# icdm-adteam/MoCoPCI

Measured on AMD Instinct MI355X. Metric: interpolated frames/sec, higher is better.
Workload: dtype f32 (fused MLP layers: fp32 products as 6 bf16-MFMA partials of an exact 3-way split, fp32 accumulate; index paths exact f32)

## Files before the change

mocopci_amd/csrc/cross.hip:

```cpp
#include "common.h"
#include "mfma_split.h"

#ifdef MCP_CROSS_DIAG
__device__ unsigned long long g_cross_diag[8];
#define CROSS_STAMP(slot)                                                                            \
    do {                                                                                             \
        unsigned long long t_;                                                                       \
        __builtin_amdgcn_sched_barrier(0);                                                           \
        asm volatile("s_memtime %0\n\ts_waitcnt lgkmcnt(0)" : "=s"(t_)::"memory");                   \
        __builtin_amdgcn_sched_barrier(0);                                                           \
        if (blockIdx.x == 0 && blockIdx.y == 0 && threadIdx.x == 0) g_cross_diag[slot] += t_ - t_prev; \
        t_prev = t_;                                                                                 \
    } while (0)
#else
#define CROSS_STAMP(slot)
#endif

namespace {

typedef float f32x16 __attribute__((ext_vector_type(16)));
constexpr int KNB = 32;
constexpr float SLOPE = 0.1f;
constexpr int MAX_MAPPED_BATCH = 1024;

__device__ __forceinline__ int chan_of(int r, int h) { return (r & 3) + 8 * (r >> 2) + 4 * h; }
__device__ __forceinline__ float leaky(float v) { return mcp_max_raw(v, v * SLOPE); }

template <int CTRL>
__device__ __forceinline__ float dppf(float v) {
    return __uint_as_float(mcp_dpp<CTRL>(__float_as_uint(v)));
}
#define MCP_MAX_DPP(dst, src0, src1, CTRL)                                                                              \
    asm("s_nop 1\n\tv_max_f32_dpp %0, %1, %2 " CTRL : "+v"(dst) : "v"(src0), "v"(src1))

__device__ __forceinline__ float scatter_max(const f32x16 &acc, int lane) {
    float v8[8], v4[4], v2[2];
#pragma unroll
    for (int r = 0; r < 8; ++r) {
        const auto sw = __builtin_amdgcn_permlane16_swap(__float_as_uint(acc[r]), __float_as_uint(acc[r + 8]), false, false);
        const float a = __uint_as_float(sw[0]), b = __uint_as_float(sw[1]);
        asm("v_max_f32 %0, %1, %2" : "=v"(v8[r]) : "v"(a), "v"(b));
    }
#pragma unroll
    for (int r = 0; r < 4; ++r) {
        float d = v8[r + 4];
        MCP_MAX_DPP(d, v8[r], v8[r], "row_ror:8 row_mask:0xf bank_mask:0x3");
        MCP_MAX_DPP(d, v8[r + 4], d, "row_ror:8 row_mask:0xf bank_mask:0xc");
        v4[r] = d;
    }
#pragma unroll
    for (int r = 0; r < 2; ++r) {
        float d = v4[r + 2];
        MCP_MAX_DPP(d, v4[r], v4[r], "row_half_mirror row_mask:0xf bank_mask:0x5");
        MCP_MAX_DPP(d, v4[r + 2], d, "row_half_mirror row_mask:0xf bank_mask:0xa");
        v2[r] = d;
    }
    const bool b1 = (lane & 2) != 0;
    float keep = b1 ? v2[1] : v2[0];
    const float send = b1 ? v2[0] : v2[1];
    MCP_MAX_DPP(keep, send, keep, "quad_perm:[2,3,0,1] row_mask:0xf bank_mask:0xf");
    MCP_MAX_DPP(keep, keep, keep, "quad_perm:[1,0,3,2] row_mask:0xf bank_mask:0xf");
    return keep;
}
__device__ __forceinline__ int scatter_reg(int lane) { return ((lane >> 4) & 1) * 8 + ((lane >> 3) & 1) * 4 + ((lane >> 2) & 1) * 2 + ((lane >> 1) & 1); }

template <int D>
struct CrossLds {
    static constexpr int T = D / 32;
    static constexpr bool BF = true;
    static constexpr int W_FLOATS = BF ? T * (2 * T) * 3 * 64 * 4 : T * (T * 16 / 4) * 64 * 4;
    static constexpr int POS_FLOATS = T * 2 * 64;
    static constexpr int B_FLOATS = T * 2 * 16;
    static constexpr int OFF_W = 0, OFF_POS = W_FLOATS, OFF_B = OFF_POS + POS_FLOATS;
    static constexpr int FLOATS = OFF_B + B_FLOATS;
};

template <int D>
__global__ __launch_bounds__(256) void cross_pack_kernel(const float *__restrict__ wpos, const float *__restrict__ bpos,
                                                         const float *__restrict__ wmlp, const float *__restrict__ bmlp,
                                                         float *__restrict__ packed) {
    using L = CrossLds<D>;
    constexpr int T = L::T, KQ = T * 4;
    for (int e = blockIdx.x * 256 + threadIdx.x; e < L::FLOATS; e += gridDim.x * 256) {
        float v;
        if (e < L::OFF_POS) {
            if (L::BF) continue;
            const int j = e & 3, lane = (e >> 2) & 63, q = (e >> 8) % KQ, t = (e >> 8) / KQ;
            const int s = 4 * q + j, tin = s >> 4, r = s & 15;
            v = wmlp[(32 * t + (lane & 31)) * D + 32 * tin + chan_of(r, lane >> 5)];
        } else if (e < L::OFF_B) {
            const int f = e - L::OFF_POS, lane = f & 63, s = (f >> 6) & 1, t = f >> 7;
            const int row = 32 * t + (lane & 31), c = 2 * s + (lane >> 5);
            v = c < 3 ? wpos[row * 3 + c] : bpos[row];
        } else {
            const int f = e - L::OFF_B, r = f & 15, h = (f >> 4) & 1, t = f >> 5;
            v = bmlp[32 * t + chan_of(r, h)];
        }
        packed[e] = v;
    }
    if (L::BF) mcp_split_weights(reinterpret_cast<uint4 *>(packed + L::OFF_W), wmlp, D, T, blockIdx.x * 256 + threadIdx.x, gridDim.x * 256);
}

template <int D>
struct CrossShape {
    static constexpr int NW = D == 128 ? 8 : 4;
    static constexpr int WG_PER_CU = D == 64 ? 3 : 1;
    static constexpr int GRID = D == 64 ? 768 : 256;
};

template <int D, int SPLIT>
__global__ __launch_bounds__(64 * CrossShape<D>::NW, CrossShape<D>::WG_PER_CU) void cross_kernel(long long total, int n1, int n2, const float *__restrict__ xyz1,
                                                           const float *__restrict__ xyz2, const float *__restrict__ points1,
                                                           const float *__restrict__ points2, const int *__restrict__ idx,
                                                           const int *__restrict__ idx2, const int *__restrict__ bmap, int shared,
                                                           const float *__restrict__ packed, float *__restrict__ out) {
    using L = CrossLds<D>;
    constexpr int T = L::T, KQ = T * 4;
    constexpr int WAVES = CrossShape<D>::NW;
    constexpr int TO = T / SPLIT;
    constexpr int WH = L::W_FLOATS / SPLIT, SMALL = L::POS_FLOATS + L::B_FLOATS;
    extern __shared__ __attribute__((aligned(16))) float lds[];
    const int tid = threadIdx.x, split = blockIdx.y;
    static_assert(WH % 4 == 0 && SMALL % 4 == 0, "LDS image is copied as float4");
    for (int e = tid; e < WH / 4; e += 64 * WAVES)
        reinterpret_cast<float4 *>(lds)[e] = reinterpret_cast<const float4 *>(packed + L::OFF_W + (size_t)split * WH)[e];
    for (int e = tid; e < SMALL / 4; e += 64 * WAVES)
        reinterpret_cast<float4 *>(lds + WH)[e] = reinterpret_cast<const float4 *>(packed + L::OFF_POS)[e];
    if (bmap) {
        const int nb = (int)(total / n1);
        for (int e = tid; e < nb; e += 64 * WAVES) reinterpret_cast<int *>(lds + WH + SMALL + WAVES * D)[e] = bmap[e];
    }
    __syncthreads();

    const int lane = tid & 63, wave = tid >> 6, h = lane >> 5, col = lane & 31;
    const float4 *wq = reinterpret_cast<const float4 *>(lds);
    const float *lpos = lds + WH, *lbias = lds + WH + L::POS_FLOATS;
    float *row1_lds = lds + WH + SMALL + wave * D;
    const int *bmap_lds = reinterpret_cast<const int *>(lds + WH + SMALL + WAVES * D);

#ifndef MCP_NO_XCD_MAP
    const bool by_xcd = gridDim.x >= 8 && (gridDim.x & 7) == 0;
#else
    const bool by_xcd = false;
#endif
    const long long chunk = by_xcd ? (total + 7) / 8 : total;
    const long long stride = (long long)(by_xcd ? gridDim.x >> 3 : gridDim.x) * WAVES;
    const long long limit = by_xcd ? min(total, ((long long)(blockIdx.x & 7) + 1) * chunk) : total;
    long long p = by_xcd ? (long long)(blockIdx.x & 7) * chunk + (long long)(blockIdx.x >> 3) * WAVES + wave : (long long)blockIdx.x * WAVES + wave;
    float q2x = 0.f, q2y = 0.f, q2z = 0.f, p1x = 0.f, p1y = 0.f, p1z = 0.f;
    float4 r1 = make_float4(0.f, 0.f, 0.f, 0.f);
    float4 rg[T][4];
    auto mapped = [&](int bb, int flag) -> long long { return (bmap && (shared & flag)) ? (long long)bmap_lds[bb] : (long long)bb; };
    struct Pos { int bb, off; };
    const int stride_b = (int)(stride / n1), stride_o = (int)(stride % n1);
    auto advance = [&](Pos q) {
        q.bb += stride_b;
        q.off += stride_o;
        if (q.off >= n1) { q.off -= n1; ++q.bb; }
        return q;
    };
    auto fetch = [&](long long pp, Pos q, int id) {
        const float *q2 = xyz2 + ((long long)q.bb * n2 + id) * 3;
        q2x = q2[0]; q2y = q2[1]; q2z = q2[2];
        p1x = xyz1[pp * 3 + 0]; p1y = xyz1[pp * 3 + 1]; p1z = xyz1[pp * 3 + 2];
        const float4 *row2 = reinterpret_cast<const float4 *>(points2 + (mapped(q.bb, 2) * n2 + id) * D);
        const float4 *row1 = reinterpret_cast<const float4 *>(points1 + (mapped(q.bb, 1) * n1 + q.off) * D);
        r1 = row1[lane < D / 4 ? lane : 0];
#pragma unroll
        for (int t = 0; t < T; ++t)
#pragma unroll
            for (int g = 0; g < 4; ++g) rg[t][g] = row2[(32 * t + 8 * g + 4 * h) >> 2];
    };
    auto nbr = [&](long long pp, Pos q) {
        if (!idx2) return idx[pp * KNB + col];
        const long long ps = mapped(q.bb, 4) * n1 + q.off;
        return col >= 16 ? idx2[pp * 16 + col - 16] : idx[ps * 16 + col];
    };
    long long pn = p + stride;
    Pos qp{(int)(p / n1), (int)(p % n1)};
    Pos qn = advance(qp), qnn = advance(qn);
    int idn = 0;
    if (p < limit) {
        fetch(p, qp, nbr(p, qp));
        if (pn < limit) idn = nbr(pn, qn);
    }
#ifdef MCP_CROSS_DIAG
    unsigned long long t_prev = 0;
    CROSS_STAMP(7);
#endif
    for (; p < limit; p = pn, pn += stride) {
        CROSS_STAMP(0);
        f32x16 x0[L::BF ? 1 : T];
        McpSplit3 xs[L::BF ? 2 * T : 1];
        const float in0 = h ? q2y - p1y : q2x - p1x, in1 = h ? 1.0f : q2z - p1z;
        if (lane < D / 4) reinterpret_cast<float4 *>(row1_lds)[lane] = r1;
        __builtin_amdgcn_wave_barrier();
#pragma unroll
        for (int t = 0; t < T; ++t) {
            f32x16 acc;
#pragma unroll
            for (int g = 0; g < 4; ++g) {
                const float4 a = reinterpret_cast<const float4 *>(row1_lds)[(32 * t + 8 * g + 4 * h) >> 2];
                acc[4 * g + 0] = a.x; acc[4 * g + 1] = a.y; acc[4 * g + 2] = a.z; acc[4 * g + 3] = a.w;
            }
            acc = __builtin_amdgcn_mfma_f32_32x32x2f32(lpos[(t * 2 + 0) * 64 + lane], in0, acc, 0, 0, 0);
            acc = __builtin_amdgcn_mfma_f32_32x32x2f32(lpos[(t * 2 + 1) * 64 + lane], in1, acc, 0, 0, 0);
#pragma unroll
            for (int g = 0; g < 4; ++g) {
                acc[4 * g + 0] = leaky(acc[4 * g + 0] + rg[t][g].x);
                acc[4 * g + 1] = leaky(acc[4 * g + 1] + rg[t][g].y);
                acc[4 * g + 2] = leaky(acc[4 * g + 2] + rg[t][g].z);
                acc[4 * g + 3] = leaky(acc[4 * g + 3] + rg[t][g].w);
            }
            if (L::BF) {
                xs[L::BF ? 2 * t : 0] = mcp_split_kstep(acc, 0);
                xs[L::BF ? 2 * t + 1 : 0] = mcp_split_kstep(acc, 1);
            } else {
                x0[L::BF ? 0 : t] = acc;
            }
        }
        __builtin_amdgcn_wave_barrier();
        CROSS_STAMP(1);
        if (pn < limit) {
            fetch(pn, qn, idn);
            if (pn + stride < limit) idn = nbr(pn + stride, qnn);
        }
        qn = qnn;
        qnn = advance(qnn);
        CROSS_STAMP(2);
#pragma unroll 1
        for (int tl = 0; tl < TO; ++tl) {
            const int t = TO * split + tl;
            f32x16 acc;
#pragma unroll
            for (int r = 0; r < 16; ++r) acc[r] = lbias[(t * 2 + h) * 16 + r];
            if (L::BF) {
                const uint4 *ws = reinterpret_cast<const uint4 *>(lds) + (size_t)tl * (2 * T) * 3 * 64 + lane;
                acc = mcp_tile_split<(L::BF ? 2 * T : 1)>(ws, xs, acc);
            } else {
#pragma unroll
                for (int q4 = 0; q4 < KQ; ++q4) {
                    const float4 w = wq[(tl * KQ + q4) * 64 + lane];
                    const int tin = L::BF ? 0 : q4 >> 2, r0 = (q4 & 3) * 4;
                    acc = __builtin_amdgcn_mfma_f32_32x32x2f32(w.x, x0[tin][r0 + 0], acc, 0, 0, 0);
                    acc = __builtin_amdgcn_mfma_f32_32x32x2f32(w.y, x0[tin][r0 + 1], acc, 0, 0, 0);
                    acc = __builtin_amdgcn_mfma_f32_32x32x2f32(w.z, x0[tin][r0 + 2], acc, 0, 0, 0);
                    acc = __builtin_amdgcn_mfma_f32_32x32x2f32(w.w, x0[tin][r0 + 3], acc, 0, 0, 0);
                }
            }
            CROSS_STAMP(3);
            const float m = leaky(scatter_max(acc, lane));
            if ((lane & 1) == 0) out[p * D + 32 * t + chan_of(scatter_reg(lane), h)] = m;
            CROSS_STAMP(4);
        }
    }
}

constexpr int X256_T = 8, X256_KS = 16, X256_TILE_U4 = X256_KS * 3 * 64, X256_WAVES = 4;
__global__ __launch_bounds__(64 * X256_WAVES, 1) void cross256_stream_kernel(long long total, int n1, int n2, const float *__restrict__ xyz1,
                                                                          const float *__restrict__ xyz2, const float *__restrict__ points1,
                                                                          const float *__restrict__ points2, const int *__restrict__ idx,
                                                                          const int *__restrict__ idx2, const int *__restrict__ bmap, int shared,
                                                                          const float *__restrict__ packed, float *__restrict__ out) {
    using L = CrossLds<256>;
// ... 167 lines not shown
```

mocopci_amd/csrc/mfma_split.h:

```cpp
#pragma once
#include "common.h"

#ifndef MCP_SPLIT_SCHED_MASK
#define MCP_SPLIT_SCHED_MASK 0x0000
#endif

typedef float mcp_f32x16 __attribute__((ext_vector_type(16)));
typedef __bf16 mcp_bf16x8 __attribute__((ext_vector_type(8)));

__device__ __forceinline__ int mcp_chan_of(int r, int h) { return (r & 3) + 8 * (r >> 2) + 4 * h; }
__device__ __forceinline__ uint32_t mcp_top16(float x) { return __float_as_uint(x) & 0xFFFF0000u; }
__device__ __forceinline__ uint32_t mcp_pack_hi(float even, float odd) {
    return __builtin_amdgcn_perm(__float_as_uint(odd), __float_as_uint(even), 0x07060302u);
}

struct McpSplit3 {
    uint4 p1, p2, p3;
};
__device__ __forceinline__ McpSplit3 mcp_split8(const float *v) {
    float r1[8], r2[8];
#pragma unroll
    for (int i = 0; i < 8; ++i) {
        r1[i] = v[i] - __uint_as_float(mcp_top16(v[i]));
        r2[i] = r1[i] - __uint_as_float(mcp_top16(r1[i]));
    }
    McpSplit3 o;
#ifdef MCP_SPLIT_DIAG_NOSPLIT
    o.p1 = make_uint4(mcp_pack_hi(v[0], v[1]), mcp_pack_hi(v[2], v[3]), mcp_pack_hi(v[4], v[5]), mcp_pack_hi(v[6], v[7]));
    o.p2 = o.p1; o.p3 = o.p1;
    return o;
#endif
    o.p1 = make_uint4(mcp_pack_hi(v[0], v[1]), mcp_pack_hi(v[2], v[3]), mcp_pack_hi(v[4], v[5]), mcp_pack_hi(v[6], v[7]));
    o.p2 = make_uint4(mcp_pack_hi(r1[0], r1[1]), mcp_pack_hi(r1[2], r1[3]), mcp_pack_hi(r1[4], r1[5]), mcp_pack_hi(r1[6], r1[7]));
    o.p3 = make_uint4(mcp_pack_hi(r2[0], r2[1]), mcp_pack_hi(r2[2], r2[3]), mcp_pack_hi(r2[4], r2[5]), mcp_pack_hi(r2[6], r2[7]));
    return o;
}
__device__ __forceinline__ McpSplit3 mcp_split_kstep(const mcp_f32x16 &a, int s) {
    float v[8];
#pragma unroll
    for (int i = 0; i < 8; ++i) v[i] = a[8 * s + i];
    return mcp_split8(v);
}
__device__ __forceinline__ mcp_f32x16 mcp_mfma_bf16(uint4 a, uint4 b, mcp_f32x16 c) {
    return __builtin_amdgcn_mfma_f32_32x32x16_bf16(__builtin_bit_cast(mcp_bf16x8, a), __builtin_bit_cast(mcp_bf16x8, b), c, 0, 0, 0);
}
__device__ __forceinline__ mcp_f32x16 mcp_mfma_split(const uint4 *w, const McpSplit3 &x, mcp_f32x16 acc) {
    const uint4 w1 = w[0], w2 = w[64], w3 = w[128];
    acc = mcp_mfma_bf16(w3, x.p1, acc);
    acc = mcp_mfma_bf16(w1, x.p3, acc);
    acc = mcp_mfma_bf16(w2, x.p2, acc);
    acc = mcp_mfma_bf16(w2, x.p1, acc);
    acc = mcp_mfma_bf16(w1, x.p2, acc);
    acc = mcp_mfma_bf16(w1, x.p1, acc);
    return acc;
}
__device__ __forceinline__ void mcp_relu_split4(const mcp_f32x16 &a, int q, McpSplit3 &o) {
    float v[4], r1[4], r2[4];
#pragma unroll
    for (int i = 0; i < 4; ++i) {
        v[i] = fmaxf(a[4 * q + i], 0.f);
        r1[i] = v[i] - __uint_as_float(mcp_top16(v[i]));
        r2[i] = r1[i] - __uint_as_float(mcp_top16(r1[i]));
    }
    const uint32_t a1 = mcp_pack_hi(v[0], v[1]), b1 = mcp_pack_hi(v[2], v[3]);
    const uint32_t a2 = mcp_pack_hi(r1[0], r1[1]), b2 = mcp_pack_hi(r1[2], r1[3]);
    const uint32_t a3 = mcp_pack_hi(r2[0], r2[1]), b3 = mcp_pack_hi(r2[2], r2[3]);
    if (q & 1) { o.p1.z = a1; o.p1.w = b1; o.p2.z = a2; o.p2.w = b2; o.p3.z = a3; o.p3.w = b3; }
    else       { o.p1.x = a1; o.p1.y = b1; o.p2.x = a2; o.p2.y = b2; o.p3.x = a3; o.p3.y = b3; }
}
template <int NF, class Fill>
__device__ __forceinline__ mcp_f32x16 mcp_kstep_fill(const uint4 &w1, const uint4 &w2, const uint4 &w3, const McpSplit3 &x, mcp_f32x16 acc, Fill fill) {
    fill();
    acc = mcp_mfma_bf16(w3, x.p1, acc);
    acc = mcp_mfma_bf16(w1, x.p3, acc);
    acc = mcp_mfma_bf16(w2, x.p2, acc);
    acc = mcp_mfma_bf16(w2, x.p1, acc);
    acc = mcp_mfma_bf16(w1, x.p2, acc);
    acc = mcp_mfma_bf16(w1, x.p1, acc);
    if constexpr (NF > 0) {
        static_assert(NF <= 30, "at most five fillers per MFMA gap");
#define MCP_GAP(i)                                                                         \
    __builtin_amdgcn_sched_group_barrier(0x008, 1, 0);                                                                                    \
    if constexpr ((NF + 5 - (i)) / 6 > 0) __builtin_amdgcn_sched_group_barrier(0x002, (NF + 5 - (i)) / 6, 0);
        MCP_GAP(0) MCP_GAP(1) MCP_GAP(2) MCP_GAP(3) MCP_GAP(4) MCP_GAP(5)
#undef MCP_GAP
    }
    __builtin_amdgcn_sched_barrier(MCP_SPLIT_SCHED_MASK);
    return acc;
}
template <int KSTEPS>
__device__ __forceinline__ mcp_f32x16 mcp_tile_split(const uint4 *ws, const McpSplit3 *xs, mcp_f32x16 acc) {
    uint4 w1 = ws[0], w2 = ws[64], w3 = ws[128];
#pragma unroll
    for (int s = 0; s < KSTEPS; ++s) {
        uint4 n1 = w1, n2 = w2, n3 = w3;
#ifndef MCP_SPLIT_DIAG_NOLOAD
        if (s + 1 < KSTEPS) {
            const uint4 *nx = ws + (size_t)(s + 1) * 3 * 64;
            n1 = nx[0]; n2 = nx[64]; n3 = nx[128];
        }
#endif
        acc = mcp_mfma_bf16(w3, xs[s].p1, acc);
        acc = mcp_mfma_bf16(w1, xs[s].p3, acc);
        acc = mcp_mfma_bf16(w2, xs[s].p2, acc);
        acc = mcp_mfma_bf16(w2, xs[s].p1, acc);
        acc = mcp_mfma_bf16(w1, xs[s].p2, acc);
        acc = mcp_mfma_bf16(w1, xs[s].p1, acc);
        __builtin_amdgcn_sched_barrier(MCP_SPLIT_SCHED_MASK);
        w1 = n1; w2 = n2; w3 = n3;
    }
    return acc;
}

__device__ __forceinline__ void mcp_split_weights(uint4 *dst, const float *__restrict__ w, int cin, int out_tiles, int first, int stride) {
    const int ksteps = cin / 16;
    for (int e = first; e < out_tiles * ksteps * 64; e += stride) {
        const int lane = e & 63, s = (e >> 6) % ksteps, t = (e >> 6) / ksteps;
        float v[8];
#pragma unroll
        for (int i = 0; i < 8; ++i) v[i] = w[(size_t)(32 * t + (lane & 31)) * cin + 32 * (s >> 1) + mcp_chan_of(8 * (s & 1) + i, lane >> 5)];
        const McpSplit3 sp = mcp_split8(v);
        uint4 *o = dst + (size_t)(t * ksteps + s) * 3 * 64 + lane;
        o[0] = sp.p1;
        o[64] = sp.p2;
        o[128] = sp.p3;
    }
}
```

mocopci_amd/csrc/fusion.hip:

```cpp
#include <stdlib.h>

#include "common.h"
#include "mfma_split.h"

namespace {

typedef float f32x16 __attribute__((ext_vector_type(16)));

constexpr int C1 = 64, C2 = 64, NB = 64;
constexpr int WAVES = 4;


__device__ __forceinline__ int chan_of(int r, int h) { return (r & 3) + 8 * (r >> 2) + 4 * h; }

__device__ __forceinline__ float wave_sum(float v) {
#pragma unroll
    for (int o = 32; o > 0; o >>= 1) v += __shfl_xor(v, o);
    return v;
}
__device__ __forceinline__ float wave_max(float v) {
#pragma unroll
    for (int o = 32; o > 0; o >>= 1) v = fmaxf(v, __shfl_xor(v, o));
    return v;
}

#ifdef MCP_AB
constexpr int OFF_W1 = 0, OFF_W2 = 256, OFF_W3 = OFF_W2 + 4096, OFF_B1 = OFF_W3 + 8192, OFF_B2 = OFF_B1 + 64,
              OFF_B3 = OFF_B2 + 64, LDS_FLOATS = OFF_B3 + 128;
__global__ __launch_bounds__(64 * WAVES, 2) void fusion_kernel(long long total, int n, const float *__restrict__ p1,
                                                            const float *__restrict__ p2, const int *__restrict__ idx, const int *__restrict__ idx2,
                                                            const float *__restrict__ w1, const float *__restrict__ b1,
                                                            const float *__restrict__ w2, const float *__restrict__ b2,
                                                            const float *__restrict__ w3, const float *__restrict__ b3,
                                                            float *__restrict__ out) {
    __shared__ __attribute__((aligned(16))) float lds[LDS_FLOATS];
    const int tid = threadIdx.x;
    for (int e = tid; e < 256; e += 64 * WAVES) {
        const int lane = e & 63, s = (e >> 6) & 1, t = e >> 7;
        lds[OFF_W1 + e] = w1[(32 * t + (lane & 31)) * 4 + 2 * s + (lane >> 5)];
    }
    for (int e = tid; e < 4096; e += 64 * WAVES) {
        const int j = e & 3, lane = (e >> 2) & 63, q = (e >> 8) & 7, t = e >> 11;
        const int s = 4 * q + j, tin = s >> 4, r = s & 15;
        lds[OFF_W2 + e] = w2[(32 * t + (lane & 31)) * C1 + 32 * tin + chan_of(r, lane >> 5)];
    }
    for (int e = tid; e < 8192; e += 64 * WAVES) {
        const int j = e & 3, lane = (e >> 2) & 63, q = (e >> 8) & 7, t = e >> 11;
        const int s = 4 * q + j, tin = s >> 4, r = s & 15;
        lds[OFF_W3 + e] = w3[(32 * t + (lane & 31)) * C2 + 32 * tin + chan_of(r, lane >> 5)];
    }
    for (int e = tid; e < 64; e += 64 * WAVES) {
        const int r = e & 15, h = (e >> 4) & 1, t = e >> 5;
        lds[OFF_B1 + e] = b1[32 * t + chan_of(r, h)];
        lds[OFF_B2 + e] = b2[32 * t + chan_of(r, h)];
    }
    for (int e = tid; e < 128; e += 64 * WAVES) {
        const int r = e & 15, h = (e >> 4) & 1, t = e >> 5;
        lds[OFF_B3 + e] = b3[32 * t + chan_of(r, h)];
    }
    __syncthreads();

    const int lane = tid & 63, wave = tid >> 6, h = lane >> 5, col = lane & 31;
    const float4 *w2q = reinterpret_cast<const float4 *>(lds + OFF_W2);
    const float4 *w3q = reinterpret_cast<const float4 *>(lds + OFF_W3);

    const McpUnits units = mcp_units_by_xcd(total, WAVES);
    for (long long p = units.first + wave; p < units.limit; p += units.stride) {
        const long long bb = mcp_div(p, n, mcp_fits32(total));
        const float cx = p1[p * 3 + 0], cy = p1[p * 3 + 1], cz = p1[p * 3 + 2];
        float score[2], nbx[2], nby[2], nbz[2];
#pragma unroll
        for (int ct = 0; ct < 2; ++ct) {
            const int id = idx2 ? (ct ? idx2 : idx)[p * 32 + col] : idx[p * NB + 32 * ct + col];
            const float *q = p2 + ((long long)bb * n + id) * 3;
            const float x = q[0], y = q[1], z = q[2];
            nbx[ct] = x; nby[ct] = y; nbz[ct] = z;
            const float rx = x - cx, ry = y - cy, rz = z - cz;
            const float dist = sqrtf((rx * rx + ry * ry) + rz * rz);
            const float in0 = h ? ry : rx, in1 = h ? dist : rz;
            f32x16 a1[2];
#pragma unroll
            for (int t = 0; t < 2; ++t) {
                f32x16 acc;
#pragma unroll
                for (int r = 0; r < 16; ++r) acc[r] = lds[OFF_B1 + (t * 2 + h) * 16 + r];
                acc = __builtin_amdgcn_mfma_f32_32x32x2f32(lds[OFF_W1 + (t * 2 + 0) * 64 + lane], in0, acc, 0, 0, 0);
                acc = __builtin_amdgcn_mfma_f32_32x32x2f32(lds[OFF_W1 + (t * 2 + 1) * 64 + lane], in1, acc, 0, 0, 0);
#pragma unroll
                for (int r = 0; r < 16; ++r) acc[r] = fmaxf(acc[r], 0.f);
                a1[t] = acc;
            }
            f32x16 a2[2];
#pragma unroll
            for (int t = 0; t < 2; ++t) {
                f32x16 acc;
#pragma unroll
                for (int r = 0; r < 16; ++r) acc[r] = lds[OFF_B2 + (t * 2 + h) * 16 + r];
#pragma unroll
                for (int q4 = 0; q4 < 8; ++q4) {
                    const float4 w = w2q[(t * 8 + q4) * 64 + lane];
                    const int tin = q4 >> 2, r0 = (q4 & 3) * 4;
                    acc = __builtin_amdgcn_mfma_f32_32x32x2f32(w.x, a1[tin][r0 + 0], acc, 0, 0, 0);
                    acc = __builtin_amdgcn_mfma_f32_32x32x2f32(w.y, a1[tin][r0 + 1], acc, 0, 0, 0);
                    acc = __builtin_amdgcn_mfma_f32_32x32x2f32(w.z, a1[tin][r0 + 2], acc, 0, 0, 0);
                    acc = __builtin_amdgcn_mfma_f32_32x32x2f32(w.w, a1[tin][r0 + 3], acc, 0, 0, 0);
                }
#pragma unroll
                for (int r = 0; r < 16; ++r) acc[r] = fmaxf(acc[r], 0.f);
                a2[t] = acc;
            }
            float m = 0.f;
#pragma unroll 1
            for (int t = 0; t < 4; ++t) {
                f32x16 acc;
#pragma unroll
                for (int r = 0; r < 16; ++r) acc[r] = lds[OFF_B3 + (t * 2 + h) * 16 + r];
#pragma unroll
                for (int q4 = 0; q4 < 8; ++q4) {
                    const float4 w = w3q[(t * 8 + q4) * 64 + lane];
                    const int tin = q4 >> 2, r0 = (q4 & 3) * 4;
                    acc = __builtin_amdgcn_mfma_f32_32x32x2f32(w.x, a2[tin][r0 + 0], acc, 0, 0, 0);
                    acc = __builtin_amdgcn_mfma_f32_32x32x2f32(w.y, a2[tin][r0 + 1], acc, 0, 0, 0);
                    acc = __builtin_amdgcn_mfma_f32_32x32x2f32(w.z, a2[tin][r0 + 2], acc, 0, 0, 0);
                    acc = __builtin_amdgcn_mfma_f32_32x32x2f32(w.w, a2[tin][r0 + 3], acc, 0, 0, 0);
                }
#pragma unroll
                for (int r = 0; r < 16; ++r) m = fmaxf(m, acc[r]);
            }
            score[ct] = fmaxf(m, __shfl_xor(m, 32));
        }
        const float mx = wave_max(fmaxf(score[0], score[1]));
        const float e0 = expf(score[0] - mx), e1 = expf(score[1] - mx);
        const float den = wave_sum(e0 + e1);
        const float sx = wave_sum(e0 * nbx[0] + e1 * nbx[1]);
        const float sy = wave_sum(e0 * nby[0] + e1 * nby[1]);
        const float sz = wave_sum(e0 * nbz[0] + e1 * nbz[1]);
        if (lane == 0) {
            out[p * 3 + 0] = sx / den;
            out[p * 3 + 1] = sy / den;
            out[p * 3 + 2] = sz / den;
        }
    }
}
#endif


constexpr int SP_W1 = 0, SP_B1 = 256, SP_B2 = SP_B1 + 64, SP_B3 = SP_B2 + 64, SP_F32_FLOATS = SP_B3 + 128;
constexpr int SP_W2_U4 = 2 * 4 * 3 * 64, SP_W3_U4 = 4 * 4 * 3 * 64;
constexpr size_t SP_LDS_BYTES = SP_F32_FLOATS * 4 + (size_t)(SP_W2_U4 + SP_W3_U4) * 16;

__device__ __forceinline__ float max4(float m, const f32x16 &a, int q) {
#pragma unroll
    for (int i = 0; i < 4; ++i) m = fmaxf(m, a[4 * q + i]);
    asm volatile("" : "+v"(m));
    return m;
}
constexpr int NF_SPLIT = 26, NF_MAX = 2;
template <int TILES, int NF0, int NF1, class Fill>
__device__ __forceinline__ void split_layer(const uint4 *wl, const float *bias, const McpSplit3 *xs, f32x16 *out, Fill fill) {
    uint4 w1 = wl[0], w2 = wl[64], w3 = wl[128];
    f32x16 acc;
#pragma unroll
    for (int i = 0; i < 16; ++i) acc[i] = bias[i];
#pragma unroll
    for (int r = 0; r < 4 * TILES; ++r) {
        uint4 n1 = w1, n2 = w2, n3 = w3;
        f32x16 nacc = acc;
        if (r + 1 < 4 * TILES) {
            const uint4 *nx = wl + (size_t)(r + 1) * 3 * 64;
            n1 = nx[0]; n2 = nx[64]; n3 = nx[128];
            if ((r & 3) == 3) {
#pragma unroll
                for (int i = 0; i < 16; ++i) nacc[i] = bias[32 * ((r >> 2) + 1) + i];
            }
        }
        if (r < 8) acc = mcp_kstep_fill<NF0>(w1, w2, w3, xs[r & 3], acc, [&] { fill(r); });
        else acc = mcp_kstep_fill<NF1>(w1, w2, w3, xs[r & 3], acc, [&] { fill(r); });
        if ((r & 3) == 3) { out[r >> 2] = acc; acc = nacc; }
        w1 = n1; w2 = n2; w3 = n3;
    }
}

__global__ __launch_bounds__(64 * WAVES, 2) void fusion_split_kernel(long long total, int n, const float *__restrict__ p1,
                                                                  const float *__restrict__ p2, const int *__restrict__ idx, const int *__restrict__ idx2,
                                                                  const float *__restrict__ w1, const float *__restrict__ b1,
                                                                  const float *__restrict__ w2, const float *__restrict__ b2,
                                                                  const float *__restrict__ w3, const float *__restrict__ b3,
                                                                  float *__restrict__ out) {
    extern __shared__ __attribute__((aligned(16))) float lds[];
    uint4 *w2s = reinterpret_cast<uint4 *>(lds + SP_F32_FLOATS);
    uint4 *w3s = w2s + SP_W2_U4;
    const int tid = threadIdx.x;
    for (int e = tid; e < 256; e += 64 * WAVES) {
        const int lane = e & 63, s = (e >> 6) & 1, t = e >> 7;
        lds[SP_W1 + e] = w1[(32 * t + (lane & 31)) * 4 + 2 * s + (lane >> 5)];
    }
    mcp_split_weights(w2s, w2, C1, 2, tid, 64 * WAVES);
    mcp_split_weights(w3s, w3, C2, 4, tid, 64 * WAVES);
    for (int e = tid; e < 64; e += 64 * WAVES) {
        const int r = e & 15, h = (e >> 4) & 1, t = e >> 5;
        lds[SP_B1 + e] = b1[32 * t + chan_of(r, h)];
        lds[SP_B2 + e] = b2[32 * t + chan_of(r, h)];
    }
    for (int e = tid; e < 128; e += 64 * WAVES) {
        const int r = e & 15, h = (e >> 4) & 1, t = e >> 5;
        lds[SP_B3 + e] = b3[32 * t + chan_of(r, h)];
    }
    __syncthreads();

    const int lane = tid & 63, wave = tid >> 6, h = lane >> 5, col = lane & 31;
    const McpUnits units = mcp_units_by_xcd(total, WAVES);
    const uint4 *w2l = w2s + lane, *w3l = w3s + lane;
    for (long long p = units.first + wave; p < units.limit; p += units.stride) {
        const long long bb = mcp_div(p, n, mcp_fits32(total));
        const float cx = p1[p * 3 + 0], cy = p1[p * 3 + 1], cz = p1[p * 3 + 2];
        float score[2], nbx[2], nby[2], nbz[2];
        f32x16 l1[2][2];
#pragma unroll
        for (int ct = 0; ct < 2; ++ct) {
            const int id = idx2 ? (ct ? idx2 : idx)[p * 32 + col] : idx[p * NB + 32 * ct + col];
            const float *q = p2 + ((long long)bb * n + id) * 3;
            const float x = q[0], y = q[1], z = q[2];
            nbx[ct] = x; nby[ct] = y; nbz[ct] = z;
            const float rx = x - cx, ry = y - cy, rz = z - cz;
            const float dist = sqrtf((rx * rx + ry * ry) + rz * rz);
            const float in0 = h ? ry : rx, in1 = h ? dist : rz;
#pragma unroll
            for (int t = 0; t < 2; ++t) {
                f32x16 acc;
#pragma unroll
                for (int r = 0; r < 16; ++r) acc[r] = lds[SP_B1 + (t * 2 + h) * 16 + r];
                acc = __builtin_amdgcn_mfma_f32_32x32x2f32(lds[SP_W1 + (t * 2 + 0) * 64 + lane], in0, acc, 0, 0, 0);
                acc = __builtin_amdgcn_mfma_f32_32x32x2f32(lds[SP_W1 + (t * 2 + 1) * 64 + lane], in1, acc, 0, 0, 0);
                l1[ct][t] = acc;
            }
        }
        McpSplit3 xa1[4], xb1[4], xa2[4], xb2[4];
        f32x16 a2[2], b2t[2], a3[4], b3t[4];
        float ma = 0.f, mb = 0.f;
#pragma unroll
        for (int u = 0; u < 8; ++u) mcp_relu_split4(l1[0][u >> 2], u & 3, xa1[u >> 1]);
        __builtin_amdgcn_sched_barrier(0);
        split_layer<2, NF_SPLIT, 0>(w2l, lds + SP_B2 + h * 16, xa1, a2, [&](int r) { if (r < 8) mcp_relu_split4(l1[1][r >> 2], r & 3, xb1[r >> 1]); });
        split_layer<2, NF_SPLIT, 0>(w2l, lds + SP_B2 + h * 16, xb1, b2t, [&](int r) { if (r < 8) mcp_relu_split4(a2[r >> 2], r & 3, xa2[r >> 1]); });
        split_layer<4, NF_SPLIT, NF_MAX>(w3l, lds + SP_B3 + h * 16, xa2, a3, [&](int r) {
            if (r < 8) mcp_relu_split4(b2t[r >> 2], r & 3, xb2[r >> 1]);
            else ma = max4(ma, a3[(r - 8) >> 2], (r - 8) & 3);
        });
        split_layer<4, NF_MAX, NF_MAX>(w3l, lds + SP_B3 + h * 16, xb2, b3t, [&](int r) {
            if (r < 8) ma = max4(ma, a3[2 + (r >> 2)], r & 3);
            else mb = max4(mb, b3t[(r - 8) >> 2], (r - 8) & 3);
        });
#pragma unroll
        for (int u = 0; u < 8; ++u) mb = max4(mb, b3t[2 + (u >> 2)], u & 3);
        score[0] = fmaxf(ma, __shfl_xor(ma, 32));
        score[1] = fmaxf(mb, __shfl_xor(mb, 32));
        const float mx = wave_max(fmaxf(score[0], score[1]));
        const float e0 = expf(score[0] - mx), e1 = expf(score[1] - mx);
        const float den = wave_sum(e0 + e1);
        const float sx = wave_sum(e0 * nbx[0] + e1 * nbx[1]);
        const float sy = wave_sum(e0 * nby[0] + e1 * nby[1]);
        const float sz = wave_sum(e0 * nbz[0] + e1 * nbz[1]);
        if (lane == 0) {
            out[p * 3 + 0] = sx / den;
            out[p * 3 + 1] = sy / den;
            out[p * 3 + 2] = sz / den;
        }
    }
}

}

MCP_EXPORT int mcp_fusion(int b, int n, int nb, const float *p1, const float *p2, const int *idx, const int *idx2, const float *w1,
                          const float *b1, const float *w2, const float *b2, const float *w3, const float *b3, float *out,
                          mcp_stream_t stream) {
    MCP_CHECK_ARGS(b > 0 && n > 0 && p1 && p2 && idx && w1 && b1 && w2 && b2 && w3 && b3 && out);
    if (nb != NB) return MCP_ERR_UNSUPPORTED;
    hipStream_t s = (hipStream_t)stream;
    const long long total = (long long)b * n;
    long long grid_cap = 4096;
#ifdef MCP_AB
    static const long long env_cap = [] { const char *v = getenv("MCP_FUSION_GRID"); return (long long)(v && *v ? atoi(v) : 0); }();
    if (env_cap >= 1) grid_cap = env_cap;
    static const bool f32_mfma = [] { const char *v = getenv("MCP_FUSION_F32_MFMA"); return v && *v == '1'; }();
#endif
    const unsigned grid = (unsigned)min((total + WAVES - 1) / WAVES, grid_cap);
    mcp_prof_begin(MCP_KERNEL_FUSION, s);
#ifdef MCP_AB
    if (f32_mfma) {
        hipLaunchKernelGGL(fusion_kernel, dim3(grid), dim3(64 * WAVES), 0, s, total, n, p1, p2, idx, idx2, w1, b1, w2, b2, w3, b3, out);
        mcp_prof_end(MCP_KERNEL_FUSION, s);
        return mcp_launch_status();
    }
#endif
    static McpPerDeviceOnce attr_once;
    if (attr_once.need()) {
        { const hipError_t attr_e_ = hipFuncSetAttribute(reinterpret_cast<const void *>(fusion_split_kernel), hipFuncAttributeMaxDynamicSharedMemorySize, 160 * 1024); if (attr_e_ != hipSuccess) return (int)attr_e_; }
        attr_once.done();
    }
    hipLaunchKernelGGL(fusion_split_kernel, dim3(grid), dim3(64 * WAVES), SP_LDS_BYTES, s, total, n, p1, p2, idx, idx2, w1, b1, w2, b2, w3, b3, out);
    mcp_prof_end(MCP_KERNEL_FUSION, s);
    return mcp_launch_status();
}
```

Measured before the change: 3719.

## Software-pipeline D=128 cross kernel, interleaving next-tile input prep with MFMA k-steps

Adds a dedicated path for the D=128, unsplit cross kernel that restructures the per-point loop into a software pipeline. The position MFMA, leaky activation and 3-way bf16 split of the next output tile's inputs are dealt out as fillers between the current tile's split-MFMA k-steps. Next-point gathers and the LDS row staging are issued one point ahead. Weight fragments are prefetched one k-step ahead from LDS. This aims to hide VALU split work and global-load latency behind the matrix pipe, at the cost of higher register pressure and a large, scheduler-barrier-heavy code path that is harder to maintain.

```diff
diff --git a/mocopci_amd/csrc/cross.hip b/mocopci_amd/csrc/cross.hip
--- a/mocopci_amd/csrc/cross.hip
+++ b/mocopci_amd/csrc/cross.hip
@@ -106,6 +106,7 @@
     static constexpr int NW = D == 128 ? 8 : 4;
     static constexpr int WG_PER_CU = D == 64 ? 3 : 1;
     static constexpr int GRID = D == 64 ? 768 : 256;
+    static constexpr bool PIPE = D == 128;
 };
 
 template <int D, int SPLIT>
@@ -180,6 +181,148 @@
     Pos qp{(int)(p / n1), (int)(p % n1)};
     Pos qn = advance(qp), qnn = advance(qn);
     int idn = 0;
+    if constexpr (CrossShape<D>::PIPE && SPLIT == 1) {
+        constexpr int NF_PAIR = 17, NF_ADD = 6, NF_SPLIT2 = 11;
+        static_assert(2 * T == 8, "a tile's eight pairs are dealt over the k-steps 1..7 of a phase");
+        auto uni = [](int v) { return __builtin_amdgcn_readfirstlane(v); };
+        p = (long long)(((unsigned long long)(unsigned)uni((int)(p >> 32)) << 32) | (unsigned)uni((int)p));
+        pn = p + stride;
+        qp = Pos{uni(qp.bb), uni(qp.off)};
+        qn = advance(qp);
+        qnn = advance(qn);
+        McpSplit3 xs[2][2];
+        float in0 = 0.f, in1 = 0.f;
+        const float4 *row2n = reinterpret_cast<const float4 *>(points2);
+        static_assert(D == 128, "the points1 row is one float2 per lane");
+        float2 r1h = make_float2(0.f, 0.f);
+        int vzero = 0;
+        asm("" : "+v"(vzero));
+        const float *q2n = xyz2, *q1n = xyz1;
+        const float2 *r1n = reinterpret_cast<const float2 *>(points1);
+        auto aim = [&](long long pp, Pos q, int id) {
+            q2n = xyz2 + ((long long)q.bb * n2 + id) * 3;
+            q1n = xyz1 + pp * 3 + vzero;
+            row2n = reinterpret_cast<const float4 *>(points2 + (mapped(q.bb, 2) * n2 + id) * D);
+            r1n = reinterpret_cast<const float2 *>(points1 + (mapped(q.bb, 1) * n1 + q.off) * D) + lane;
+        };
+        auto fetch_head = [&] {
+            q2x = q2n[0]; q2y = q2n[1]; q2z = q2n[2];
+            p1x = q1n[0]; p1y = q1n[1]; p1z = q1n[2];
+            r1h = *r1n;
+        };
+        auto fetch_tile = [&](int t) {
+#pragma unroll
+            for (int g = 0; g < 4; ++g) rg[t][g] = row2n[(32 * t + 8 * g + 4 * h) >> 2];
+        };
+        auto put_point = [&] {
+            asm volatile("" : "+v"(q2x), "+v"(q2y), "+v"(q2z), "+v"(p1x), "+v"(p1y), "+v"(p1z), "+v"(r1h.x), "+v"(r1h.y));
+            in0 = h ? q2y - p1y : q2x - p1x;
+            in1 = h ? 1.0f : q2z - p1z;
+            reinterpret_cast<float2 *>(row1_lds)[lane] = r1h;
+            __builtin_amdgcn_wave_barrier();
+        };
+        f32x16 brow;
+        float lp0 = 0.f, lp1 = 0.f;
+        auto read_row = [&](int t) {
+#pragma unroll
+            for (int g = 0; g < 4; ++g) {
+                const float4 a = reinterpret_cast<const float4 *>(row1_lds)[(32 * t + 8 * g + 4 * h) >> 2];
+                brow[4 * g + 0] = a.x; brow[4 * g + 1] = a.y; brow[4 * g + 2] = a.z; brow[4 * g + 3] = a.w;
+            }
+            lp0 = lpos[(t * 2 + 0) * 64 + lane];
+            lp1 = lpos[(t * 2 + 1) * 64 + lane];
+        };
+        auto pos_tile = [&] {
+            f32x16 b = __builtin_amdgcn_mfma_f32_32x32x2f32(lp0, in0, brow, 0, 0, 0);
+            b = __builtin_amdgcn_mfma_f32_32x32x2f32(lp1, in1, b, 0, 0, 0);
+            return b;
+        };
+        auto x0_pair = [&](const f32x16 &b, int t, int j, float &v0, float &v1) {
+            const float4 g = rg[t][j >> 1];
+            const float s0 = b[2 * j] + ((j & 1) ? g.z : g.x), s1 = b[2 * j + 1] + ((j & 1) ? g.w : g.y);
+            v0 = fmaxf(s0, s0 * SLOPE);
+            v1 = fmaxf(s1, s1 * SLOPE);
+        };
+        if (p < limit) {
+            const int id = nbr(p, qp);
+            if (pn < limit) idn = nbr(pn, qn);
+            aim(p, qp, id);
+            fetch_head();
+#pragma unroll
+            for (int t = 0; t < T; ++t) fetch_tile(t);
+            put_point();
+            read_row(0);
+            const f32x16 b = pos_tile();
+#pragma unroll
+            for (int j = 0; j < 8; ++j) {
+                float v0, v1;
+                x0_pair(b, 0, j, v0, v1);
+                mcp_split2(v0, v1, j & 3, xs[0][j >> 2]);
+            }
+            read_row(1);
+        }
+        int far = 4096;
+        asm("" : "+v"(far));
+        const uint4 *wl = reinterpret_cast<const uint4 *>(lds) + lane, *wl_far = wl + far;
+        auto piece = [&](int e) { return e < 4096 ? wl[e] : wl_far[e - 4096]; };
+        uint4 w1 = wl[0], w2 = wl[64], w3 = wl[128];
+        for (; p < limit; p = pn, pn += stride) {
+            const bool more = pn < limit;
+            if (more) {
+                aim(pn, qn, idn);
+                if (pn + stride < limit) idn = nbr(pn + stride, qnn);
+            }
+            fetch_head();
+            fetch_tile(0);
+            f32x16 acc[T];
+#pragma unroll
+            for (int t = 0; t < T; ++t)
+#pragma unroll
+                for (int r = 0; r < 16; ++r) acc[t][r] = lbias[(t * 2 + h) * 16 + r];
+            __builtin_amdgcn_sched_barrier(0);
+#pragma unroll
+            for (int t = 0; t < T; ++t) {
+                const int nt = (t + 1) % T;
+                if (t > 0) fetch_tile(t);
+                const f32x16 b = pos_tile();
+                __builtin_amdgcn_sched_barrier(0);
+                McpSplit3 *xn = xs[(t + 1) & 1];
+                float l0 = 0.f, l1 = 0.f;
+#pragma unroll
+                for (int s = 0; s < 2 * T; ++s) {
+                    const int to = s % T, kh = s / T;
+                    const int s2 = (s + 1) % (2 * T), t2 = s + 1 < 2 * T ? t : nt;
+                    const int nx = (((s2 % T) * 2 * T + 2 * t2 + s2 / T) * 3) * 64;
+                    const uint4 n1 = piece(nx), n2 = piece(nx + 64), n3 = piece(nx + 128);
+                    auto pair = [&](int j) {
+                        float v0, v1;
+                        x0_pair(b, nt, j, v0, v1);
+                        mcp_split2(v0, v1, j & 3, xn[j >> 2]);
+                    };
+                    if (s == 0 && t == T - 2) put_point();
+                    if (s == 2 * T - 1) read_row((t + 2) % T);
+                    const McpSplit3 &x = xs[t & 1][kh];
+                    if (s == 0) acc[to] = mcp_kstep_fill<0>(w1, w2, w3, x, acc[to], [] {});
+                    else if (s < 2 * T - 2) acc[to] = mcp_kstep_fill<NF_PAIR>(w1, w2, w3, x, acc[to], [&] { pair(s - 1); });
+                    else if (s == 2 * T - 2) acc[to] = mcp_kstep_fill<NF_PAIR + NF_ADD>(w1, w2, w3, x, acc[to], [&] { pair(5); x0_pair(b, nt, 7, l0, l1); });
+                    else acc[to] = mcp_kstep_fill<NF_PAIR + NF_SPLIT2>(w1, w2, w3, x, acc[to], [&] { pair(6); mcp_split2(l0, l1, 3, xn[1]); });
+                    w1 = n1; w2 = n2; w3 = n3;
+                }
+            }
+#pragma unroll
+            for (int k = 0; k < 2; ++k)
+                asm volatile("" ::"v"(xs[0][k].p1.x), "v"(xs[0][k].p1.y), "v"(xs[0][k].p1.z), "v"(xs[0][k].p1.w), "v"(xs[0][k].p2.x), "v"(xs[0][k].p2.y),
+                             "v"(xs[0][k].p2.z), "v"(xs[0][k].p2.w), "v"(xs[0][k].p3.x), "v"(xs[0][k].p3.y), "v"(xs[0][k].p3.z), "v"(xs[0][k].p3.w));
+#pragma unroll
+            for (int t = 0; t < T; ++t) {
+                const float m = leaky(scatter_max(acc[t], lane));
+                if ((lane & 1) == 0) out[p * D + 32 * t + chan_of(scatter_reg(lane), h)] = m;
+            }
+            qn = qnn;
+            qnn = advance(qnn);
+        }
+        return;
+    }
     if (p < limit) {
         fetch(p, qp, nbr(p, qp));
         if (pn < limit) idn = nbr(pn, qn);
diff --git a/mocopci_amd/csrc/mfma_split.h b/mocopci_amd/csrc/mfma_split.h
--- a/mocopci_amd/csrc/mfma_split.h
+++ b/mocopci_amd/csrc/mfma_split.h
@@ -68,6 +68,17 @@
     if (q & 1) { o.p1.z = a1; o.p1.w = b1; o.p2.z = a2; o.p2.w = b2; o.p3.z = a3; o.p3.w = b3; }
     else       { o.p1.x = a1; o.p1.y = b1; o.p2.x = a2; o.p2.y = b2; o.p3.x = a3; o.p3.y = b3; }
 }
+__device__ __forceinline__ void mcp_split2(float v0, float v1, int j, McpSplit3 &o) {
+    const float a1 = v0 - __uint_as_float(mcp_top16(v0)), b1 = v1 - __uint_as_float(mcp_top16(v1));
+    const float a2 = a1 - __uint_as_float(mcp_top16(a1)), b2 = b1 - __uint_as_float(mcp_top16(b1));
+    const uint32_t d1 = mcp_pack_hi(v0, v1), d2 = mcp_pack_hi(a1, b1), d3 = mcp_pack_hi(a2, b2);
+    switch (j) {
+        case 0: o.p1.x = d1; o.p2.x = d2; o.p3.x = d3; break;
+        case 1: o.p1.y = d1; o.p2.y = d2; o.p3.y = d3; break;
+        case 2: o.p1.z = d1; o.p2.z = d2; o.p3.z = d3; break;
+        default: o.p1.w = d1; o.p2.w = d2; o.p3.w = d3; break;
+    }
+}
 template <int NF, class Fill>
 __device__ __forceinline__ mcp_f32x16 mcp_kstep_fill(const uint4 &w1, const uint4 &w2, const uint4 &w3, const McpSplit3 &x, mcp_f32x16 acc, Fill fill) {
     fill();
```

New measurement: 3724 (median of 4 runs). About the same (+0.1%).

## Software-pipeline fusion kernel across points and use DPP/permlane reductions

Applied to the files above, without the earlier changes.

Restructures the per-wave point loop into a software pipeline. The next point's neighbour indices and coordinates are prefetched, its layer-1 MFMAs and ReLU splits are interleaved into the current point's layer-3 MFMA schedule, and the previous point's softmax reduction tail and store are deferred into the next iteration. Shuffle-based wave reductions are replaced with DPP and permlane swap sequences, and the per-point batch division is replaced by incremental index advancement. This hides memory latency and the scalar tail behind matrix work, at the cost of higher register pressure and intricate hand-tuned fill schedules.

```diff
diff --git a/mocopci_amd/csrc/fusion.hip b/mocopci_amd/csrc/fusion.hip
--- a/mocopci_amd/csrc/fusion.hip
+++ b/mocopci_amd/csrc/fusion.hip
@@ -22,6 +22,35 @@
 #pragma unroll
     for (int o = 32; o > 0; o >>= 1) v = fmaxf(v, __shfl_xor(v, o));
     return v;
+}
+
+template <int CTRL, int BANKS>
+__device__ __forceinline__ float dpp_move(float old, float v) {
+    return __int_as_float(__builtin_amdgcn_update_dpp(__float_as_int(old), __float_as_int(v), CTRL, 0xF, BANKS, false));
+}
+__device__ __forceinline__ float wave_sum_reg(float v) {
+    const auto a = __builtin_amdgcn_permlane32_swap(__float_as_uint(v), __float_as_uint(v), false, false);
+    v = __uint_as_float(a[0]) + __uint_as_float(a[1]);
+    const auto b = __builtin_amdgcn_permlane16_swap(__float_as_uint(v), __float_as_uint(v), false, false);
+    v = __uint_as_float(b[0]) + __uint_as_float(b[1]);
+    v += dpp_move<0x128, 0xF>(v, v);
+    v += dpp_move<0x114, 0xA>(dpp_move<0x104, 0x5>(v, v), v);
+    v += dpp_move<0x4E, 0xF>(v, v);
+    v += dpp_move<0xB1, 0xF>(v, v);
+    return v;
+}
+__device__ __forceinline__ float wave_max_reg(float v) {
+    v = fmaxf(v, dpp_move<0xB1, 0xF>(v, v));
+    v = fmaxf(v, dpp_move<0x4E, 0xF>(v, v));
+    v = fmaxf(v, dpp_move<0x141, 0xF>(v, v));
+    v = fmaxf(v, dpp_move<0x140, 0xF>(v, v));
+    v = fmaxf(v, __int_as_float(__builtin_amdgcn_update_dpp(__float_as_int(v), __float_as_int(v), 0x142, 0xA, 0xF, false)));
+    v = fmaxf(v, __int_as_float(__builtin_amdgcn_update_dpp(__float_as_int(v), __float_as_int(v), 0x143, 0xC, 0xF, false)));
+    return __int_as_float(__builtin_amdgcn_readlane(__float_as_int(v), 63));
+}
+__device__ __forceinline__ float half_max_reg(float v) {
+    const auto a = __builtin_amdgcn_permlane32_swap(__float_as_uint(v), __float_as_uint(v), false, false);
+    return fmaxf(__uint_as_float(a[0]), __uint_as_float(a[1]));
 }
 
 #ifdef MCP_AB
@@ -155,31 +184,58 @@
     asm volatile("" : "+v"(m));
     return m;
 }
+__device__ __forceinline__ void keep_split4(McpSplit3 &o, int q) {
+    if (q & 1) asm volatile("" : "+v"(o.p1.z), "+v"(o.p1.w), "+v"(o.p2.z), "+v"(o.p2.w), "+v"(o.p3.z), "+v"(o.p3.w));
+    else asm volatile("" : "+v"(o.p1.x), "+v"(o.p1.y), "+v"(o.p2.x), "+v"(o.p2.y), "+v"(o.p3.x), "+v"(o.p3.y));
+}
 constexpr int NF_SPLIT = 26, NF_MAX = 2;
-template <int TILES, int NF0, int NF1, class Fill>
-__device__ __forceinline__ void split_layer(const uint4 *wl, const float *bias, const McpSplit3 *xs, f32x16 *out, Fill fill) {
+template <int R>
+struct Step {
+    static constexpr int value = R;
+};
+template <int R, int N, class F>
+__device__ __forceinline__ void static_for(F &f) {
+    if constexpr (R < N) {
+        f(Step<R>{});
+        static_for<R + 1, N>(f);
+    }
+}
+template <int TILES, class Sched, class Fill, class Pre>
+__device__ __forceinline__ void split_layer(const uint4 *wl, const float *bias, const McpSplit3 *xs, f32x16 *out, Fill fill, Pre pre) {
     uint4 w1 = wl[0], w2 = wl[64], w3 = wl[128];
     f32x16 acc;
 #pragma unroll
     for (int i = 0; i < 16; ++i) acc[i] = bias[i];
-#pragma unroll
-    for (int r = 0; r < 4 * TILES; ++r) {
+    auto step = [&](auto rc) {
+        constexpr int r = decltype(rc)::value;
+        pre(rc);
         uint4 n1 = w1, n2 = w2, n3 = w3;
         f32x16 nacc = acc;
-        if (r + 1 < 4 * TILES) {
+        if constexpr (r + 1 < 4 * TILES) {
             const uint4 *nx = wl + (size_t)(r + 1) * 3 * 64;
             n1 = nx[0]; n2 = nx[64]; n3 = nx[128];
-            if ((r & 3) == 3) {
+            if constexpr ((r & 3) == 3) {
 #pragma unroll
                 for (int i = 0; i < 16; ++i) nacc[i] = bias[32 * ((r >> 2) + 1) + i];
             }
         }
-        if (r < 8) acc = mcp_kstep_fill<NF0>(w1, w2, w3, xs[r & 3], acc, [&] { fill(r); });
-        else acc = mcp_kstep_fill<NF1>(w1, w2, w3, xs[r & 3], acc, [&] { fill(r); });
-        if ((r & 3) == 3) { out[r >> 2] = acc; acc = nacc; }
+        acc = mcp_kstep_fill<Sched::nf(r)>(w1, w2, w3, xs[r & 3], acc, [&] { fill(rc); });
+        if constexpr ((r & 3) == 3) { out[r >> 2] = acc; acc = nacc; }
         w1 = n1; w2 = n2; w3 = n3;
-    }
-}
+    };
+    static_for<0, 4 * TILES>(step);
+}
+constexpr int NF_DIFF = 8, NF_ROOT = 18;
+struct SchedSplit {
+    static constexpr int nf(int r) { return NF_SPLIT; }
+};
+constexpr int NF_TAIL[8] = {26, 28, 20, 22, 22, 22, 22, 11};
+struct SchedA3 {
+    static constexpr int nf(int r) { return r < 5 ? NF_SPLIT : r < 8 ? NF_SPLIT + NF_MAX : NF_MAX + NF_TAIL[r - 8]; }
+};
+struct SchedB3 {
+    static constexpr int nf(int r) { return r < 4 ? NF_MAX + ((r & 1) ? NF_ROOT : NF_DIFF) : r < 8 ? NF_MAX : NF_MAX + NF_SPLIT; }
+};
 
 __global__ __launch_bounds__(64 * WAVES, 2) void fusion_split_kernel(long long total, int n, const float *__restrict__ p1,
                                                                   const float *__restrict__ p2, const int *__restrict__ idx, const int *__restrict__ idx2,
@@ -211,62 +267,138 @@
     const int lane = tid & 63, wave = tid >> 6, h = lane >> 5, col = lane & 31;
     const McpUnits units = mcp_units_by_xcd(total, WAVES);
     const uint4 *w2l = w2s + lane, *w3l = w3s + lane;
-    for (long long p = units.first + wave; p < units.limit; p += units.stride) {
-        const long long bb = mcp_div(p, n, mcp_fits32(total));
-        const float cx = p1[p * 3 + 0], cy = p1[p * 3 + 1], cz = p1[p * 3 + 2];
-        float score[2], nbx[2], nby[2], nbz[2];
-        f32x16 l1[2][2];
-#pragma unroll
-        for (int ct = 0; ct < 2; ++ct) {
-            const int id = idx2 ? (ct ? idx2 : idx)[p * 32 + col] : idx[p * NB + 32 * ct + col];
-            const float *q = p2 + ((long long)bb * n + id) * 3;
-            const float x = q[0], y = q[1], z = q[2];
-            nbx[ct] = x; nby[ct] = y; nbz[ct] = z;
-            const float rx = x - cx, ry = y - cy, rz = z - cz;
-            const float dist = sqrtf((rx * rx + ry * ry) + rz * rz);
-            const float in0 = h ? ry : rx, in1 = h ? dist : rz;
-#pragma unroll
-            for (int t = 0; t < 2; ++t) {
-                f32x16 acc;
-#pragma unroll
-                for (int r = 0; r < 16; ++r) acc[r] = lds[SP_B1 + (t * 2 + h) * 16 + r];
-                acc = __builtin_amdgcn_mfma_f32_32x32x2f32(lds[SP_W1 + (t * 2 + 0) * 64 + lane], in0, acc, 0, 0, 0);
-                acc = __builtin_amdgcn_mfma_f32_32x32x2f32(lds[SP_W1 + (t * 2 + 1) * 64 + lane], in1, acc, 0, 0, 0);
-                l1[ct][t] = acc;
-            }
+    long long p = units.first + wave, pn = p + units.stride;
+    if (p >= units.limit) return;
+    const bool fits32 = mcp_fits32(total);
+    int bbn = (int)mcp_div(p, n, fits32), offn = (int)(p - (long long)bbn * n);
+    const int stride_b = (int)mcp_div(units.stride, n, fits32), stride_o = (int)(units.stride - (long long)stride_b * n);
+    auto advance = [&] {
+        bbn += stride_b;
+        offn += stride_o;
+        if (offn >= n) { offn -= n; ++bbn; }
+    };
+    auto nbr = [&](long long pp, int ct) { return idx2 ? (ct ? idx2 : idx)[pp * 32 + col] : idx[pp * NB + 32 * ct + col]; };
+    struct Raw {
+        float cx, cy, cz, x0, y0, z0, x1, y1, z1;
+    };
+    auto fetch = [&](long long pp, int id0, int id1) {
+        const float *qa = p2 + ((long long)bbn * n + id0) * 3, *qb = p2 + ((long long)bbn * n + id1) * 3;
+        return Raw{p1[pp * 3 + 0], p1[pp * 3 + 1], p1[pp * 3 + 2], qa[0], qa[1], qa[2], qb[0], qb[1], qb[2]};
+    };
+    float rx, ry, rz, ss;
+    auto diff = [&](float x, float y, float z, const Raw &c) {
+        rx = x - c.cx; ry = y - c.cy; rz = z - c.cz;
+        ss = (rx * rx + ry * ry) + rz * rz;
+    };
+    auto root = [&](float &in0, float &in1) {
+        const float dist = sqrtf(ss);
+        in0 = h ? ry : rx; in1 = h ? dist : rz;
+    };
+    auto l1_bias = [&](int t) {
+        f32x16 acc;
+#pragma unroll
+        for (int r = 0; r < 16; ++r) acc[r] = lds[SP_B1 + (t * 2 + h) * 16 + r];
+        return acc;
+    };
+    auto l1_w = [&](int t, int s) { return lds[SP_W1 + (t * 2 + s) * 64 + lane]; };
+    auto l1_tile = [&](f32x16 acc, float wa, float wb, float in0, float in1) {
+        acc = __builtin_amdgcn_mfma_f32_32x32x2f32(wa, in0, acc, 0, 0, 0);
+        return __builtin_amdgcn_mfma_f32_32x32x2f32(wb, in1, acc, 0, 0, 0);
+    };
+
+    Raw cur = fetch(p, nbr(p, 0), nbr(p, 1)), nxt = cur;
+    advance();
+    int idn0 = 0, idn1 = 0;
+    if (pn < units.limit) { idn0 = nbr(pn, 0); idn1 = nbr(pn, 1); }
+    float in0a, in1a, in0b, in1b;
+    McpSplit3 xa1[4];
+    diff(cur.x0, cur.y0, cur.z0, cur); root(in0a, in1a);
+    diff(cur.x1, cur.y1, cur.z1, cur); root(in0b, in1b);
+    {
+        f32x16 l1a[2];
+#pragma unroll
+        for (int t = 0; t < 2; ++t) l1a[t] = l1_tile(l1_bias(t), l1_w(t, 0), l1_w(t, 1), in0a, in1a);
+#pragma unroll
+        for (int u = 0; u < 8; ++u) mcp_relu_split4(l1a[u >> 2], u & 3, xa1[u >> 1]);
+    }
+    struct Tail {
+        float ma, mb, x0, y0, z0, x1, y1, z1;
+        long long p;
+    } prev = {0.f, 0.f, 0.f, 0.f, 0.f, 0.f, 0.f, 0.f, -1};
+    float s0, s1, mx, e0, e1, den, sx, sy, sz, ox = 0.f, oy = 0.f, oz = 0.f;
+    auto tail = [&](auto kc) {
+        constexpr int k = decltype(kc)::value;
+        if constexpr (k == 0) { s0 = half_max_reg(prev.ma); s1 = half_max_reg(prev.mb); mx = wave_max_reg(fmaxf(s0, s1)); }
+        if constexpr (k == 1) { e0 = expf(s0 - mx); e1 = expf(s1 - mx); }
+        if constexpr (k == 2) den = wave_sum_reg(e0 + e1);
+        if constexpr (k == 3) sx = wave_sum_reg(e0 * prev.x0 + e1 * prev.x1);
+        if constexpr (k == 4) sy = wave_sum_reg(e0 * prev.y0 + e1 * prev.y1);
+        if constexpr (k == 5) sz = wave_sum_reg(e0 * prev.z0 + e1 * prev.z1);
+        if constexpr (k == 6) { ox = sx / den; oy = sy / den; }
+        if constexpr (k == 7) { oz = sz / den; asm volatile("" : "+v"(ox), "+v"(oy), "+v"(oz)); }
+    };
+    auto store = [&] {
+        if (lane == 0 && prev.p >= 0) {
+            out[prev.p * 3 + 0] = ox;
+            out[prev.p * 3 + 1] = oy;
+            out[prev.p * 3 + 2] = oz;
         }
-        McpSplit3 xa1[4], xb1[4], xa2[4], xb2[4];
+    };
+    for (; p < units.limit; p = pn, pn += units.stride) {
+        if (pn < units.limit) {
+            nxt = fetch(pn, idn0, idn1);
+            if (pn + units.stride < units.limit) { idn0 = nbr(pn + units.stride, 0); idn1 = nbr(pn + units.stride, 1); }
+        }
+        advance();
+        f32x16 l1b[2];
+#pragma unroll
+        for (int t = 0; t < 2; ++t) l1b[t] = l1_tile(l1_bias(t), l1_w(t, 0), l1_w(t, 1), in0b, in1b);
+        __builtin_amdgcn_sched_barrier(0);
+        McpSplit3 xb1[4], xa2[4], xb2[4];
         f32x16 a2[2], b2t[2], a3[4], b3t[4];
         float ma = 0.f, mb = 0.f;
-#pragma unroll
-        for (int u = 0; u < 8; ++u) mcp_relu_split4(l1[0][u >> 2], u & 3, xa1[u >> 1]);
-        __builtin_amdgcn_sched_barrier(0);
-        split_layer<2, NF_SPLIT, 0>(w2l, lds + SP_B2 + h * 16, xa1, a2, [&](int r) { if (r < 8) mcp_relu_split4(l1[1][r >> 2], r & 3, xb1[r >> 1]); });
-        split_layer<2, NF_SPLIT, 0>(w2l, lds + SP_B2 + h * 16, xb1, b2t, [&](int r) { if (r < 8) mcp_relu_split4(a2[r >> 2], r & 3, xa2[r >> 1]); });
-        split_layer<4, NF_SPLIT, NF_MAX>(w3l, lds + SP_B3 + h * 16, xa2, a3, [&](int r) {
-            if (r < 8) mcp_relu_split4(b2t[r >> 2], r & 3, xb2[r >> 1]);
-            else ma = max4(ma, a3[(r - 8) >> 2], (r - 8) & 3);
+        auto none = [](auto) {};
+        split_layer<2, SchedSplit>(w2l, lds + SP_B2 + h * 16, xa1, a2, [&](auto rc) {
+            constexpr int r = decltype(rc)::value;
+            mcp_relu_split4(l1b[r >> 2], r & 3, xb1[r >> 1]);
+        }, none);
+        split_layer<2, SchedSplit>(w2l, lds + SP_B2 + h * 16, xb1, b2t, [&](auto rc) {
+            constexpr int r = decltype(rc)::value;
+            mcp_relu_split4(a2[r >> 2], r & 3, xa2[r >> 1]);
+        }, none);
+        split_layer<4, SchedA3>(w3l, lds + SP_B3 + h * 16, xa2, a3, [&](auto rc) {
+            constexpr int r = decltype(rc)::value;
+            if constexpr (r < 8) mcp_relu_split4(b2t[r >> 2], r & 3, xb2[r >> 1]);
+            if constexpr (r >= 5) ma = max4(ma, a3[(r - 5) >> 2], (r - 5) & 3);
+            if constexpr (r >= 8) tail(Step<r - 8>{});
+        }, none);
+        float in0n = 0.f, in1n = 0.f, nwa = 0.f, nwb = 0.f;
+        f32x16 nl1[2], nbias;
+        split_layer<4, SchedB3>(w3l, lds + SP_B3 + h * 16, xb2, b3t, [&](auto rc) {
+            constexpr int r = decltype(rc)::value;
+            if constexpr (r < 5) ma = max4(ma, a3[(r + 11) >> 2], (r + 11) & 3);
+            else mb = max4(mb, b3t[(r - 5) >> 2], (r - 5) & 3);
+            if constexpr (r == 0) diff(nxt.x0, nxt.y0, nxt.z0, nxt);
+            if constexpr (r == 1) root(in0n, in1n);
+            if constexpr (r == 2) diff(nxt.x1, nxt.y1, nxt.z1, nxt);
+            if constexpr (r == 3) { root(in0b, in1b); asm volatile("" : "+v"(in0b), "+v"(in1b)); }
+            if constexpr (r >= 8) { mcp_relu_split4(nl1[(r - 8) >> 2], (r - 8) & 3, xa1[(r - 8) >> 1]); keep_split4(xa1[(r - 8) >> 1], (r - 8) & 3); }
+        }, [&](auto rc) {
+            constexpr int r = decltype(rc)::value;
+            if constexpr (r == 6 || r == 10) { nbias = l1_bias(r == 10); nwa = l1_w(r == 10, 0); nwb = l1_w(r == 10, 1); }
+            if constexpr (r == 7 || r == 11) {
+                nl1[r == 11] = l1_tile(nbias, nwa, nwb, in0n, in1n);
+                __builtin_amdgcn_sched_barrier(0);
+            }
         });
-        split_layer<4, NF_MAX, NF_MAX>(w3l, lds + SP_B3 + h * 16, xb2, b3t, [&](int r) {
-            if (r < 8) ma = max4(ma, a3[2 + (r >> 2)], r & 3);
-            else mb = max4(mb, b3t[(r - 8) >> 2], (r - 8) & 3);
-        });
-#pragma unroll
-        for (int u = 0; u < 8; ++u) mb = max4(mb, b3t[2 + (u >> 2)], u & 3);
-        score[0] = fmaxf(ma, __shfl_xor(ma, 32));
-        score[1] = fmaxf(mb, __shfl_xor(mb, 32));
-        const float mx = wave_max(fmaxf(score[0], score[1]));
-        const float e0 = expf(score[0] - mx), e1 = expf(score[1] - mx);
-        const float den = wave_sum(e0 + e1);
-        const float sx = wave_sum(e0 * nbx[0] + e1 * nbx[1]);
-        const float sy = wave_sum(e0 * nby[0] + e1 * nby[1]);
-        const float sz = wave_sum(e0 * nbz[0] + e1 * nbz[1]);
-        if (lane == 0) {
-            out[p * 3 + 0] = sx / den;
-            out[p * 3 + 1] = sy / den;
-            out[p * 3 + 2] = sz / den;
-        }
-    }
+#pragma unroll
+        for (int u = 11; u < 16; ++u) mb = max4(mb, b3t[u >> 2], u & 3);
+        store();
+        prev = Tail{ma, mb, cur.x0, cur.y0, cur.z0, cur.x1, cur.y1, cur.z1, p};
+        cur = nxt;
+    }
+    static_for<0, 8>(tail);
+    store();
 }
 
 }
```

Result: no change. 3697 before, 3707 after (median of 3 runs) (+0.3%).
